# WestlyPark/StyleRenderer

Measured on AMD Instinct MI355X. Metric: generator fwd+bwd images/sec at 256^2, higher is better.
Workload: dtype f32

## Files before the change

### include/stylerenderer_amd.h

```cpp
#ifndef STYLERENDERER_AMD_H_
#define STYLERENDERER_AMD_H_

#include <stddef.h>
#include <stdint.h>

#ifdef __cplusplus
extern "C" {
#endif

typedef void* sr_stream_t;

#define SR_OK 0
#define SR_EINVAL (-1)
#define SR_ERANGE (-2)

const char* sr_error_string(int code);
int sr_abi_version(void);

int sr_fused_bias_act(float* y, const float* x, const float* b, const float* ref, int act, int grad,
                      float alpha, float scale, int64_t size_x, int64_t step_b, int64_t size_b,
                      int use_bias, int use_ref, sr_stream_t stream);

int64_t sr_fused_act_bwd_scratch_floats(int64_t n, int64_t c, int64_t inner);
int sr_fused_act_bwd(float* gx, float* gb, const float* gy, const float* out, float alpha,
// ... 194 lines not shown
                              float eps, sr_stream_t stream);
int sr_rasterize_backward_f64(int64_t b, int64_t n, int64_t h, int64_t w, int repeat_v,
                              int perspective, const double* v, const int64_t* index,
                              double* dcoeff, double eps, sr_stream_t stream);

int64_t sr_rasterize_grad_scratch_bytes(int64_t b, int64_t nf, int64_t tex_c, int is_double);
int sr_rasterize_grad_f32(int64_t b, int64_t nv, int64_t nf, int64_t h, int64_t w, int repeat_f,
                          int perspective, const float* v, const float* tex, int64_t tex_c,
                          const int64_t* tri, const int32_t* win, const int32_t* big, const float* grad_out,
                          const int32_t* adj_off, const int32_t* adj, int64_t adj_off_bstride,
                          int64_t adj_bstride, const int32_t* adj_slot, float* grad_v, float* grad_tex, float eps,
                          void* work, sr_stream_t stream);
int sr_rasterize_grad_f64(int64_t b, int64_t nv, int64_t nf, int64_t h, int64_t w, int repeat_f,
                          int perspective, const double* v, const double* tex, int64_t tex_c,
                          const int64_t* tri, const int32_t* win, const int32_t* big, const double* grad_out,
                          const int32_t* adj_off, const int32_t* adj, int64_t adj_off_bstride,
                          int64_t adj_bstride, const int32_t* adj_slot, double* grad_v, double* grad_tex, double eps,
                          void* work, sr_stream_t stream);

int sr_rasterize_forward_cpu_f32(int64_t b, int64_t nv, int64_t nf, int64_t h, int64_t w, int repeat_v,
                                 int repeat_f, int perspective, const float* v, const int64_t* tri,
                                 int64_t* index, float* coeff, float* zbuf, float eps);
int sr_rasterize_forward_cpu_f64(int64_t b, int64_t nv, int64_t nf, int64_t h, int64_t w, int repeat_v,
                                 int repeat_f, int perspective, const double* v, const int64_t* tri,
                                 int64_t* index, double* coeff, double* zbuf, double eps);
int sr_rasterize_backward_cpu_f32(int64_t b, int64_t n, int64_t h, int64_t w, int perspective,
                                  const float* v, const int64_t* index, float* dcoeff, float eps);
int sr_rasterize_backward_cpu_f64(int64_t b, int64_t n, int64_t h, int64_t w, int perspective,
                                  const double* v, const int64_t* index, double* dcoeff, double eps);

int64_t sr_conv2d_scratch_floats(int64_t B, int64_t C, int64_t N, int64_t IH, int64_t IW, int64_t OH,
                                 int64_t OW, int ksize, int stride, int pad, int transposed);
int sr_conv2d_mfma(float* out, const float* in, const float* wt, const float* iscale,
                   const float* oscale, const float* obias, int64_t B, int64_t C, int64_t N,
                   int64_t wt_ld, int64_t IH, int64_t IW, int64_t OH, int64_t OW, int ksize, int stride,
                   int pad, int transposed, float* scratch, sr_stream_t stream);
int sr_conv2d_nba(float* out, const float* in, const float* wt, const float* iscale, const float* oscale,
                  const float* noise, const float* noise_w, const float* abias, float alpha, float gain, int64_t B,
                  int64_t C, int64_t N, int64_t wt_ld, int64_t H, int64_t W, int64_t noise_bstride, float* scratch,
                  sr_stream_t stream);

#define SR_CONV_U_READY 1
int sr_conv2d_uses_winograd(int64_t B, int64_t C, int64_t N, int64_t IH, int64_t IW, const float* in, const float* out);
#define SR_CONV_PATH_INVALID (-1)
#define SR_CONV_PATH_DIRECT 0
#define SR_CONV_PATH_WINO 1
#define SR_CONV_PATH_S2_BF16 2
#define SR_CONV_PATH_S2_WINO 3
#define SR_CONV_PATH_GEMM1X1 4
#define SR_CONV_PATH_CONVT_TAPS 5
#define SR_CONV_PATH_CONVT_BF16 6
#define SR_CONV_PATH_CONVT_FUSED_KS 7
#define SR_CONV_PATH_CONVT_FUSED 8
#define SR_CONV_PATH_STRIPS 0x100
int sr_conv2d_path(int64_t B, int64_t C, int64_t N, int64_t IH, int64_t IW, int64_t OH, int64_t OW, int ksize, int stride,
                   int pad, int transposed, const float* in, const float* out, const float* wt, int64_t wt_ld,
                   int have_scratch);
int64_t sr_conv2d_path_floats(int64_t B, int64_t C, int64_t N, int64_t IH, int64_t IW, int64_t OH, int64_t OW, int ksize,
                              int stride, int pad, int transposed, const float* in, const float* out, const float* wt,
                              int64_t wt_ld, int have_scratch);

int sr_conv2d_generic(float* y, const float* x, const float* w, const float* bias, int64_t B, int64_t C, int64_t N,
                      int64_t IH, int64_t IW, int64_t OH, int64_t OW, int kh, int kw, int sy, int sx, int py, int px,
                      sr_stream_t stream);
int sr_conv2d_generic_dgrad(float* dx, const float* g, const float* w, int64_t B, int64_t C, int64_t N, int64_t IH,
                            int64_t IW, int64_t OH, int64_t OW, int kh, int kw, int sy, int sx, int py, int px,
                            sr_stream_t stream);
int sr_conv2d_generic_wgrad(float* dw, const float* x, const float* g, int64_t B, int64_t C, int64_t N, int64_t IH,
                            int64_t IW, int64_t OH, int64_t OW, int kh, int kw, int sy, int sx, int py, int px,
                            sr_stream_t stream);
int sr_conv2d_mfma_ex(float* out, const float* in, const float* wt, const float* iscale,
                      const float* oscale, const float* obias, int64_t B, int64_t C, int64_t N,
                      int64_t wt_ld, int64_t IH, int64_t IW, int64_t OH, int64_t OW, int ksize,
                      int stride, int pad, int transposed, int flags, float* scratch, sr_stream_t stream);
int sr_conv1x1_add_supported(int64_t B, int64_t C, int64_t N, int64_t wt_ld, int64_t P, const float* in, const float* wt,
                             const float* out, const float* addend);
int sr_conv1x1_add(float* out, const float* in, const float* wt, const float* oscale, const float* addend, int64_t B,
                   int64_t C, int64_t N, int64_t wt_ld, int64_t P, sr_stream_t stream);
int sr_conv2d_nba_ex(float* out, const float* in, const float* wt, const float* iscale, const float* oscale,
                     const float* noise, const float* noise_w, const float* abias, float alpha, float gain,
                     int64_t B, int64_t C, int64_t N, int64_t wt_ld, int64_t H, int64_t W, int64_t noise_bstride,
                     int flags, float* scratch, sr_stream_t stream);

int64_t sr_conv2d_wgrad_scratch_floats(int64_t B, int64_t C, int64_t N, int64_t IH, int64_t IW,
                                       int64_t OH, int64_t OW, int ksize, int stride, int pad,
                                       int transposed);
int sr_conv2d_wgrad_mfma(float* dwt, const float* x, const float* gy, const float* xscale,
                         const float* gscale, int64_t B, int64_t C, int64_t N, int64_t IH,
                         int64_t IW, int64_t OH, int64_t OW, int ksize, int stride, int pad,
                         int transposed, float* scratch, sr_stream_t stream);
#define SR_WGRAD_PATH_INVALID (-1)
#define SR_WGRAD_PATH_DIRECT 0
#define SR_WGRAD_PATH_SMALL3 1
#define SR_WGRAD_PATH_WINO 2
#define SR_WGRAD_PATH_BF16_1X1 3
#define SR_WGRAD_PATH_BF16_S2 4
#define SR_WGRAD_PATH_S2_DMA 5
#define SR_WGRAD_PATH_S2_WINO 6
int sr_conv2d_wgrad_path(int64_t B, int64_t C, int64_t N, int64_t IH, int64_t IW, int64_t OH, int64_t OW, int ksize,
                         int stride, int pad, int transposed, const float* x, const float* gy);
int64_t sr_conv2d_wgrad_path_floats(int64_t B, int64_t C, int64_t N, int64_t IH, int64_t IW, int64_t OH, int64_t OW,
                                    int ksize, int stride, int pad, int transposed, const float* x, const float* gy);

int sr_signal_bump(uint32_t* counter, sr_stream_t stream);
int sr_signal_set(uint32_t* word, const uint32_t* epoch, sr_stream_t stream);
int sr_signal_wait(const uint32_t* counter, uint32_t at_least, sr_stream_t stream);
// ... 113 lines not shown
```

### stylerenderer_amd/_lib.py

```python
import ctypes
import os

_HERE = os.path.dirname(os.path.abspath(__file__))
LIB_PATH = os.environ.get("STYLERENDERER_AMD_LIB") or os.path.join(_HERE, "libstylerenderer_hip.so")

_i = ctypes.c_int
_l = ctypes.c_int64
_f = ctypes.c_float
_d = ctypes.c_double
_p = ctypes.c_void_p

SIGNATURES = {
    "sr_error_string": (ctypes.c_char_p, [_i]),
    "sr_abi_version": (_i, []),
    "sr_fused_bias_act": (_i, [_p, _p, _p, _p, _i, _i, _f, _f, _l, _l, _l, _i, _i, _p]),
    "sr_fused_act_bwd_scratch_floats": (_l, [_l, _l, _l]),
    "sr_fused_act_bwd": (_i, [_p, _p, _p, _p, _f, _f, _l, _l, _l, _p, _p]),
    "sr_noise_bias_act": (_i, [_p] * 6 + [_f, _f] + [_l] * 4 + [_p]),
    "sr_noise_bias_act_bwd_scratch_floats": (_l, [_l, _l, _l]),
    "sr_noise_bias_act_bwd": (_i, [_p] * 6 + [_f, _f] + [_l] * 4 + [_p, _p]),
    "sr_noise_bias_act_bwd_dot_scratch_floats": (_l, [_l, _l, _l]),
    "sr_noise_bias_act_bwd_dot": (_i, [_p] * 9 + [_f, _f] + [_l] * 4 + [_p, _p]),
    "sr_conv2d_nba": (_i, [_p] * 8 + [_f, _f] + [_l] * 7 + [_p, _p]),
    "sr_conv2d_nba_ex": (_i, [_p] * 8 + [_f, _f] + [_l] * 7 + [_i, _p, _p]),
# ... 89 lines not shown
    "sr_conv2d_mfma_ex": (_i, [_p] * 6 + [_l] * 8 + [_i] * 5 + [_p, _p]),
    "sr_conv1x1_add_supported": (_i, [_l] * 5 + [_p] * 4),
    "sr_conv1x1_add": (_i, [_p] * 5 + [_l] * 5 + [_p]),
    "sr_rasterize_grad_f64": (_i, [_l] * 5 + [_i] * 2 + [_p, _p, _l] + [_p] * 6 + [_l, _l, _p, _p, _p, _d, _p, _p]),
    "sr_pose_fwd": (_i, [_p, _p, _p, _p]),
    "sr_pose_bwd": (_i, [_p, _p, _p, _p, _p]),
    "sr_pose_batch_fwd": (_i, [_p, _p, _p, _l, _p]),
    "sr_affine3_fwd": (_i, [_p, _p, _p, _p, _l, _l, _l, _p]),
    "sr_affine3_bwd": (_i, [_p, _p, _p, _p, _l, _l, _l, _p]),
    "sr_morph_fwd": (_i, [_p] * 9 + [_f, _l, _l, _l, _p]),
    "sr_vertex_normals_bwd_f32": (_i, [_p] * 11 + [_l, _l, _l, _f, _p]),
    "sr_morph_gcoeff_scratch_floats": (_l, [_l, _l, _l]),
    "sr_morph_gcoeff": (_i, [_p] * 6 + [_f, _p, _l, _l, _l, _p]),
    "sr_morph_pose_bwd": (_i, [_p] * 5 + [_l, _p]),
    "sr_skin_joints_fwd": (_i, [_p] * 11 + [_f] + [_l] * 4 + [_p]),
    "sr_skin_fwd": (_i, [_p] * 7 + [_l] * 4 + [_p]),
    "sr_skin_bwd_scratch_floats": (_l, [_l, _l, _l]),
    "sr_skin_bwd": (_i, [_p] * 7 + [_l] * 3 + [_p]),
    "sr_skin_joints_bwd": (_i, [_p] * 11 + [_f, _p] + [_l] * 5 + [_p]),
    "sr_blend_z_floats": (_l, [_l, _l, _l]),
    "sr_blend_head": (_i, [_p] * 6 + [_f] + [_l] * 3 + [_p]),
    "sr_blend_fwd": (_i, [_p] * 8 + [_l] * 4 + [_p]),
    "sr_blend_gz": (_i, [_p] * 3 + [_l] * 4 + [_p]),
    "sr_blend_tail": (_i, [_p] * 5 + [_f, _p] + [_l] * 3 + [_p]),
    "sr_resample_u8_scratch_bytes": (_l, [_l] * 6 + [ctypes.POINTER(ctypes.c_int32)] + [_l] * 4),
    "sr_resample_u8": (_i, [_p, _p] + [_l] * 6 + [_p, _p, ctypes.POINTER(ctypes.c_int32), _l] * 2 + [_l] * 4
                       + [_i, _i, _p, _p]),
    "sr_warp_affine_u8": (_i, [_p, _p, _p] + [_l] * 7 + [_i, _i, _i, _p]),
    "sr_landmark_loss_fwd": (_i, [_p] * 8 + [_l] * 5 + [_f, _f, _p]),
    "sr_landmark_loss_bwd": (_i, [_p, _p, _p, _l, _p, _p, _p] + [_l] * 5 + [_i, _p]),
    "sr_landmark_dyn_fwd": (_i, [_p] * 15 + [_l] * 6 + [_i, _f, _f, _l, _l, _f, _f, _p]),
    "sr_landmark_dyn_bwd": (_i, [_p, _p, _p, _l] + [_p] * 7 + [_l] * 6 + [_i, _p]),
    "sr_region_fill": (_i, [_p, _p, _p] + [_l] * 6 + [_p]),
    "sr_region_grow": (_i, [_p, _p, _l, _l, _l, _i, _p]),
    "sr_region_blend_fwd": (_i, [_p] * 6 + [_l] * 4 + [_f] + [_l] * 4 + [_p]),
    "sr_region_blend_bwd": (_i, [_p] * 3 + [_l] * 4 + [_p]),
    "sr_texture_bake": (_i, [_p] * 9 + [_l] * 10 + [_f, _f, _f, _p]),
    "sr_texture_pad": (_i, [_p] * 4 + [_l] * 4 + [_p]),
    "sr_texture_merge": (_i, [_p] * 5 + [_l] * 4 + [_i, _p]),
    "sr_share_rows": (_i, [_p] + [_l] * 3 + [_p]),
    "sr_camera_fwd": (_i, [_p] * 5 + [_l, _l, _p]),
    "sr_camera_bwd": (_i, [_p] * 6 + [_l, _l, _p]),
    "sr_signal_bump": (_i, [_p, _p]),
    "sr_signal_wait": (_i, [_p, ctypes.c_uint32, _p]),
    "sr_signal_set": (_i, [_p, _p, _p]),
    "sr_signal_set_host": (_i, [_p, _p, _p]),
    "sr_signal_wait_timeout": (_i, [_p, ctypes.c_uint32, ctypes.c_uint64, _p, _i, _p]),
    "sr_signal_wait_poison": (_i, [_p, ctypes.c_uint32, ctypes.c_uint64, _p, _i, _p, _p]),
    "sr_graph_replace_memset_nodes": (_i, [_p, ctypes.POINTER(_i)]),
    "sr_graph_node_count": (_i, [_p, ctypes.POINTER(_i), ctypes.POINTER(_i)]),
}

(CONV_PATH_DIRECT, CONV_PATH_WINO, CONV_PATH_S2_BF16, CONV_PATH_S2_WINO, CONV_PATH_GEMM1X1, CONV_PATH_CONVT_TAPS,
 CONV_PATH_CONVT_BF16, CONV_PATH_CONVT_FUSED_KS, CONV_PATH_CONVT_FUSED) = range(9)
CONV_PATH_STRIPS = 0x100
(WGRAD_PATH_DIRECT, WGRAD_PATH_SMALL3, WGRAD_PATH_WINO, WGRAD_PATH_BF16_1X1, WGRAD_PATH_BF16_S2,
 WGRAD_PATH_S2_DMA, WGRAD_PATH_S2_WINO) = range(7)

_lib = None


class NativeLibraryError(RuntimeError):
    pass


def lib():
    global _lib
    if _lib is not None:
        return _lib
    if not os.path.isfile(LIB_PATH):
        raise NativeLibraryError(
            "stylerenderer_amd: %s not found. Build it with `python -c 'import __graft_entry__ as g; "
            "g.build()'` (hipcc --offload-arch=gfx950). There is no CPU/PyTorch fallback for device "
            "tensors." % LIB_PATH)
    try:
        handle = ctypes.CDLL(LIB_PATH)
    except OSError as e:
        raise NativeLibraryError("stylerenderer_amd: cannot load %s: %s" % (LIB_PATH, e))
    for name, (res, args) in SIGNATURES.items():
        try:
            fn = getattr(handle, name)
        except AttributeError:
            raise NativeLibraryError("stylerenderer_amd: %s does not export %s" % (LIB_PATH, name))
        fn.restype = res
        fn.argtypes = args
    _lib = handle
    return _lib


def check(rc, what=""):
    if rc != 0:
        msg = lib().sr_error_string(rc)
        raise RuntimeError("%s failed: %s (code %d)" % (what or "stylerenderer_amd call",
                                                        msg.decode() if msg else "?", rc))


def ptr(t):
    if t is None or t.numel() == 0:
        return None
    return t.data_ptr()


def current_stream(device=None):
    import torch

    return torch.cuda.current_stream(device).cuda_stream
```

### stylerenderer_amd/build.py

```python
import os
import subprocess
import sys

HERE = os.path.dirname(os.path.abspath(__file__))
CSRC = os.path.join(HERE, "csrc")
LIB = os.path.join(HERE, "libstylerenderer_hip.so")
OBJ = os.path.join(HERE, "csrc", "_obj")

ARCH = "gfx950"
COMMON = ["--offload-arch=" + ARCH, "-O3", "-std=c++17", "-fPIC", "-Wno-unused-result",
          "-fhip-fp32-correctly-rounded-divide-sqrt"]
EXACT = ["-ffp-contract=off"]
NOSLP = ["-fno-slp-vectorize"]

SOURCES = [
    ("capi.hip", EXACT),
    ("fused_bias_act.hip", EXACT),
    ("upfirdn2d.hip", EXACT + NOSLP),
    ("rasterize.hip", EXACT),
    ("fused_elem.hip", EXACT),
    ("weight_prep.hip", EXACT),
    ("style_linear.hip", EXACT),
    ("bank_mm.hip", EXACT),
    ("mesh.hip", EXACT),
    ("landmark.hip", EXACT),
    ("region.hip", EXACT),
    ("texture.hip", EXACT),
    ("share.hip", EXACT),
    ("camera.hip", EXACT),
    ("morph.hip", []),
    ("skin.hip", []),
    ("blend.hip", []),
    ("lpips.hip", EXACT),
    ("ppl.hip", EXACT),
    ("augment.hip", EXACT),
    ("resample.hip", EXACT),
    ("warp.hip", EXACT),
    ("conv_mfma.hip", []),
    ("conv_wino.hip", []),
    ("conv_wgrad_wino.hip", []),
    ("conv_wgrad_mfma.hip", []),
    ("conv_wgrad_bf16x3.hip", []),
    ("conv_wgrad_s2_wino.hip", []),
    ("conv_s2_bf16x3.hip", []),
    ("conv_s2_wino.hip", []),
    ("conv_generic.hip", []),
    ("conv1x1_gemm.hip", []),
    ("inception.hip", []),
]


def _hipcc():
    for c in (os.environ.get("HIPCC"), "/opt/rocm/bin/hipcc", "hipcc"):
        if c and (os.path.isabs(c) and os.path.exists(c) or not os.path.isabs(c)):
            return c
    return "hipcc"


def _deps(src):
    deps = [src, os.path.join(CSRC, "common.h"),
            os.path.join(HERE, "..", "include", "stylerenderer_amd.h"), os.path.abspath(__file__)]
    deps += [os.path.join(CSRC, f) for f in os.listdir(CSRC) if f.endswith(".h")]
    return max(os.path.getmtime(d) for d in deps if os.path.exists(d))


def build_library(force=False, verbose=False):
    os.makedirs(OBJ, exist_ok=True)
    hipcc = _hipcc()
    objs, rebuilt = [], False
    procs = []
    for name, extra in SOURCES:
        src = os.path.join(CSRC, name)
        obj = os.path.join(OBJ, name.replace(".hip", ".o"))
        objs.append(obj)
        if force or not os.path.exists(obj) or os.path.getmtime(obj) < _deps(src):
            cmd = [hipcc] + COMMON + extra + ["-c", src, "-o", obj]
            if verbose:
                print(" ".join(cmd))
            procs.append((name, subprocess.Popen(cmd, stdout=subprocess.PIPE, stderr=subprocess.STDOUT)))
            rebuilt = True
    for name, p in procs:
        out, _ = p.communicate()
        if p.returncode != 0:
            sys.stderr.write(out.decode(errors="replace"))
            raise RuntimeError("hipcc failed on %s" % name)
        if verbose and out:
            sys.stdout.write(out.decode(errors="replace"))
    if rebuilt or not os.path.exists(LIB):
        cmd = [hipcc, "--offload-arch=" + ARCH, "-shared", "-fPIC", "-o", LIB] + objs
        if verbose:
            print(" ".join(cmd))
        subprocess.check_call(cmd)
    return LIB


if __name__ == "__main__":
    print(build_library(force="-f" in sys.argv, verbose=True))
```

### stylerenderer_amd/csrc/conv_mfma.hip

```cpp
#include "common.h"
#include "conv1x1_gemm.h"
#include "conv_s2_bf16x3.h"
#include "conv_s2_wino.h"
#include "conv_wgrad_bf16x3.h"
#include "conv_wino.h"

#include <algorithm>
#include <cstdlib>

namespace {

typedef float f32x16 __attribute__((ext_vector_type(16)));
typedef const void __attribute__((address_space(1)))* gptr_t;
typedef void __attribute__((address_space(3)))* lptr_t;

constexpr int BN = 128;
constexpr int BM = 128;

__device__ __attribute__((aligned(16))) const float g_zero_line[4] = {0.f, 0.f, 0.f, 0.f};
__device__ __attribute__((aligned(16))) const float g_ones_line[4] = {1.f, 1.f, 1.f, 1.f};

struct ConvParams {
    const float* in;
    const float* wt;
    const float* iscale;
    const float* oscale;
    const float* obias;
    float* out;
    int B, C, N, ldw;
    int IH, IW;
    int GH, GW;
    int gy_base, gx_base;
    int OH, OW;
    int osy, osx, ooy, oox;
    int dy0, dx0;
    int wmap[9];
    int tiles_x, tiles_y, tiles_b, tiles_n;
    float* partial;
    int64_t partial_floats;
    int ks, c_per_slice;
    int tap_first, tap_step, tap_count;
};

template <int IS, int TY, int TX, int PW, int PH, int PB, bool V4, bool TAP9 = false>
struct Geo {
    static constexpr bool ROT = V4 && IS == 2;
    static constexpr int NT = TY * TX;
    static constexpr int KC = NT >= 9 ? 4 : (NT >= 4 ? 8 : 16);
    static constexpr int EH = (PH - 1) * IS + TY;
    static constexpr int EW = (PW - 1) * IS + TX;
    static constexpr int LEAD = (V4 && !ROT) ? (TAP9 ? 4 : (TX > 1 ? 3 : 0)) : 0;
    static constexpr int EWP = ROT ? (EW + 3 + 3) / 4 * 4
                                   : (V4 ? (LEAD + EW + 3) / 4 * 4 : EW + ((EW % 2 == 0) ? 1 : 0));
    static constexpr int PLANE = PB * EH * EWP;
    static constexpr int W_FLOATS = NT * KC * BN;
    static constexpr int W_INSTR = W_FLOATS / 256;
    static constexpr int IMG_INSTR = V4 ? (KC * PLANE + 255) / 256 : 0;
    static constexpr int ST_INSTR = V4 ? (KC * PB + 63) / 64 : 0;
// ... 813 lines not shown
    if (ext_w <= 0 || ext_h <= 0) return SR_OK;
    choose_split(ext_h, ext_w, p.B, p.N, p.C, p.ks, p.c_per_slice);
    if (!p.partial || (int64_t)p.ks * p.B * p.N * ext_h * ext_w > p.partial_floats) {
        p.ks = 1;
        p.c_per_slice = (p.C + 15) / 16 * 16;
    }
    patch_shape(ext_w, pw, ph, pb);
    p.tiles_x = (ext_w + pw - 1) / pw;
    p.tiles_y = (ext_h + ph - 1) / ph;
    p.tiles_b = (p.B + pb - 1) / pb;
    p.tiles_n = (p.N + BN - 1) / BN;
    const int64_t blocks = (int64_t)p.tiles_x * p.tiles_y * p.tiles_b * p.tiles_n * p.ks;
    if (blocks <= 0) return SR_OK;
    if (blocks > 0x7FFFFFFFLL) return SR_ERANGE;
    const dim3 grid((unsigned)blocks);
    const bool v4 = IS == 1 && pb == 1 && p.IW % 4 == 0 && sr_aligned16(p.in) &&
                    p.gx_base % 4 == 0 && p.dx0 == (TX > 1 ? -1 : 0);
    const bool rot = IS == 2 && pb == 1 && (p.IW & 3) == 1 && ((p.IH * p.IW) & 3) == 1 && p.C % 4 == 0 &&
                     sr_aligned16(p.in) && p.dx0 >= 0 && p.dy0 >= 0 && p.gx_base == 0 &&
                     p.gy_base == 0 && (p.GW - 1) * 2 + p.dx0 + TX <= p.IW && (p.GH - 1) * 2 + p.dy0 + TY <= p.IH &&
                     ext_w % pw == 0 && ext_h % ph == 0 && !sr_env_off("SR_CONV_ROT");
    int rc;
    if (IS == 1 && v4) {
        if (pw == 32) rc = launch_one<1, TY, TX, 32, 4, 1, true>(p, grid, st);
        else rc = launch_one<1, TY, TX, 16, 8, 1, true>(p, grid, st);
    } else if (IS == 2 && rot && TY == 3 && TX == 3) {
        if (pw == 32) rc = launch_one<2, 3, 3, 32, 4, 1, true>(p, grid, st);
        else rc = launch_one<2, 3, 3, 16, 8, 1, true>(p, grid, st);
    } else if (pw == 32) rc = launch_one<IS, TY, TX, 32, 4, 1, false>(p, grid, st);
    else if (pw == 16) rc = launch_one<IS, TY, TX, 16, 8, 1, false>(p, grid, st);
    else if (pw == 8) rc = launch_one<IS, TY, TX, 8, 8, 2, false>(p, grid, st);
    else rc = launch_one<IS, TY, TX, 4, 4, 8, false>(p, grid, st);
    if (rc != SR_OK || p.ks <= 1) return rc;
    const int64_t total = (int64_t)p.B * p.N * ext_h * ext_w;
    hipLaunchKernelGGL(k_conv_reduce, dim3(sr_stream_grid(total, 256)), dim3(256), 0, st, p, ext_h, ext_w);
    return sr_launch_status();
}


int64_t direct_floats(const ConvCall& c) {
    int ks, per;
    int64_t need = 0;
    auto consider = [&](int64_t gh, int64_t gw) {
        if (gh <= 0 || gw <= 0) return;
        choose_split((int)gh, (int)gw, (int)c.B, (int)c.N, (int)c.C, ks, per);
        if (ks > 1) need = std::max(need, ks * c.B * c.N * gh * gw);
    };
    if (!c.transposed) consider(c.OH, c.OW);
    else consider(c.IH + 1, c.IW + 1), consider(c.IH, c.IW), consider(1, c.IW + 1), consider(c.IH, 1);
    return need;
}

bool convt_interior(int path) {
    return path == SR_CONV_PATH_CONVT_BF16 || path == SR_CONV_PATH_CONVT_FUSED_KS || path == SR_CONV_PATH_CONVT_FUSED;
}

struct ConvPlan {
    int path = SR_CONV_PATH_DIRECT;
    bool strips = false;
    int ks = 1, c_per_slice = 0;
    bool taps_gemm = false;
    int64_t floats = 0;
    int64_t sized = 0;
    int code() const { return path | (strips ? SR_CONV_PATH_STRIPS : 0); }
};

ConvPlan make_conv_plan(const ConvCall& c, bool have_scratch) {
    ConvPlan plan;
    const int64_t B = c.B, C = c.C, N = c.N, IH = c.IH, IW = c.IW, OH = c.OH, OW = c.OW;
    if (B <= 0 || C <= 0 || N <= 0 || OH <= 0 || OW <= 0) return plan;
    plan.sized = plan.floats = direct_floats(c);
    auto candidate = [&](int path, bool reach, bool take, int64_t floats, int ks = 1) {
        if (!reach) return;
        plan.sized = std::max(plan.sized, floats);
        if (plan.path != SR_CONV_PATH_DIRECT || !take || (floats > 0 && !have_scratch)) return;
        plan.path = path; plan.floats = floats; plan.ks = ks;
    };
    if (!c.transposed && c.is3x3(1, 1)) {
        if (sr_winograd_enabled() && sr_wino_eligible(B, C, N, IH, IW, nullptr, nullptr))
            candidate(SR_CONV_PATH_WINO, true, sr_wino_eligible(B, C, N, IH, IW, c.in, c.out),
                      sr_wino_scratch_floats(C, N) + sr_wino_partial_floats(B, C, N, IH, IW));
    } else if (!c.transposed && c.is3x3(2, 0)) {
        candidate(SR_CONV_PATH_S2_BF16, sr_wgrad_bf16x3_enabled('c') && sr_conv_s2_bf16x3_eligible(B, C, N, IH, IW, OH, OW),
                  true, sr_conv_s2_bf16x3_scratch_floats(C, N));
        const int sw = sr_env_char("SR_CONV_S2_WINO");
        candidate(SR_CONV_PATH_S2_WINO, sr_conv_s2_wino_eligible(B, C, N, IH, IW, OH, OW, nullptr, nullptr),
                  sw != '0' && sr_conv_s2_wino_eligible(B, C, N, IH, IW, OH, OW, c.in, c.out) &&
                      (sw == 'f' || sr_conv_s2_wino_blocks(B, N, OH, OW) >= S2_WINO_MIN_BLOCKS),
                  sr_conv_s2_wino_scratch_floats(C, N));
    } else if (!c.transposed && c.ksize == 1 && c.stride == 1) {
        candidate(SR_CONV_PATH_GEMM1X1, true,
                  c.pad == 0 && sr_conv1x1_gemm_eligible(B, C, N, c.ldw, IH * IW, c.in, c.wt, c.out), 0);
    } else if (c.transposed && c.is3x3(2, 0)) {
        const bool bf = sr_wgrad_bf16x3_enabled('t') && sr_convt_bf16x3_eligible(B, C, N, IH, IW);
        if (convt_taps_wanted(B, C, N, IH, IW)) {
            int ks;
            convt_taps_plan((int)IH, (int)IW, (int)B, (int)N, (int)C, ks, plan.c_per_slice);
            candidate(SR_CONV_PATH_CONVT_TAPS, true, !bf, (int64_t)ks * 9 * B * N * (IH + 1) * (IW + 1), ks);
        }
        candidate(SR_CONV_PATH_CONVT_BF16, bf, true, sr_convt_bf16x3_scratch_floats(C, N));
        const int sw = sr_env_char("SR_CONVT_FUSED");
        const bool fused_ok = sw != '0' && IW >= 16 && convt_fused_eligible(c);
        const int64_t blocks = (IW / TFused::PW) * (IH / TFused::PH) * ((N + BN - 1) / BN) * B;
        const bool pays = blocks >= 192 || C <= 256;
        const int ks = (IW % TFused::PW || IH % TFused::PH || pays) ? 1 : convt_fused_slices(blocks, (int)C);
        candidate(SR_CONV_PATH_CONVT_FUSED_KS, ks > 1, fused_ok && !sr_env_off("SR_CONVT_FUSED_KS"),
                  ks * B * N * (2 * IH + 1) * (2 * IW + 1), ks);
        candidate(SR_CONV_PATH_CONVT_FUSED, true, fused_ok && (pays || sw == '1'), 0);
        const int64_t strip = convt_strip_floats(B, N, IH, IW);
        plan.sized = std::max(plan.sized, strip);
        if (convt_interior(plan.path) && have_scratch && !sr_env_off("SR_CONVT_STRIPS")) {
            plan.strips = true;
            plan.floats = std::max(plan.floats, strip);
        }
    }
    if (plan.path == SR_CONV_PATH_CONVT_TAPS)
        plan.taps_gemm = sr_convt_taps_gemm_eligible(B, C, N, IW, c.ldw, plan.c_per_slice, c.wt);
    return plan;
}

bool conv_call_valid(const ConvCall& c) {
    if (c.B < 0 || c.C <= 0 || c.N <= 0 || c.IH <= 0 || c.IW <= 0 || c.OH <= 0 || c.OW <= 0) return false;
    if (c.transposed) return c.is3x3(2, 0) && c.OH == 2 * c.IH + 1 && c.OW == 2 * c.IW + 1;
    return (c.ksize == 3 || c.ksize == 1) && (c.stride == 1 || c.stride == 2) &&
           c.OH == (c.IH + 2 * c.pad - c.ksize) / c.stride + 1 && c.OW == (c.IW + 2 * c.pad - c.ksize) / c.stride + 1;
}

int launch_convt_phases(ConvParams p, bool interior_done, hipStream_t st) {
    for (int py = 0; py < 2; ++py)
        for (int px = 0; px < 2; ++px) {
            const int TYp = py == 0 ? 2 : 1, TXp = px == 0 ? 2 : 1;
            p.osy = p.osx = 2; p.ooy = py; p.oox = px;
            p.dy0 = -(TYp - 1); p.dx0 = -(TXp - 1);
            for (int ty = 0; ty < TYp; ++ty)
                for (int tx = 0; tx < TXp; ++tx) {
                    const int ky = py + 2 * (TYp - 1 - ty), kx = px + 2 * (TXp - 1 - tx);
                    p.wmap[ty * TXp + tx] = ky * 3 + kx;
                }
            const int gh_full = py == 0 ? p.IH + 1 : p.IH, gw_full = px == 0 ? p.IW + 1 : p.IW;
            int regions[3][4] = {{0, p.IH, 0, p.IW},
                                 {p.IH, gh_full, 0, gw_full},
                                 {0, p.IH, p.IW, gw_full}};
            const bool split_border = p.IW >= 16;
            if (!split_border) {
                regions[0][1] = gh_full;
                regions[0][3] = gw_full;
            }
            const bool fused = split_border && interior_done;
            for (int rg = fused ? 1 : 0; rg < (split_border ? 3 : 1); ++rg) {
                p.gy_base = regions[rg][0]; p.GH = regions[rg][1];
                p.gx_base = regions[rg][2]; p.GW = regions[rg][3];
                if (p.GH <= p.gy_base || p.GW <= p.gx_base) continue;
                int rc;
                if (py == 0 && px == 0) rc = launch_by_patch<1, 2, 2>(p, st);
// ... 25 lines not shown
extern "C" int64_t sr_conv2d_path_floats(int64_t B, int64_t C, int64_t N, int64_t IH, int64_t IW, int64_t OH, int64_t OW,
                                         int ksize, int stride, int pad, int transposed, const float* in, const float* out,
                                         const float* wt, int64_t wt_ld, int have_scratch) {
    const ConvCall c{B, C, N, IH, IW, OH, OW, ksize, stride, pad, transposed, in, out, wt, wt_ld};
    return conv_call_valid(c) ? make_conv_plan(c, have_scratch != 0).floats : -1;
}

extern "C" int sr_conv2d_uses_winograd(int64_t B, int64_t C, int64_t N, int64_t IH, int64_t IW, const float* in,
                                       const float* out) {
    return make_conv_plan(ConvCall{B, C, N, IH, IW, IH, IW, 3, 1, 1, 0, in, out, nullptr, 0}, true).path == SR_CONV_PATH_WINO;
}

extern "C" int sr_conv2d_mfma_ex(float* out, const float* in, const float* wt, const float* iscale,
                              const float* oscale, const float* obias, int64_t B, int64_t C,
                              int64_t N, int64_t wt_ld, int64_t IH, int64_t IW, int64_t OH, int64_t OW,
                              int ksize, int stride, int pad, int transposed, int flags, float* scratch,
                              sr_stream_t stream) {
    const ConvCall c{B, C, N, IH, IW, OH, OW, ksize, stride, pad, transposed, in, out, wt, wt_ld};
    if (B < 0 || C <= 0 || N <= 0 || IH <= 0 || IW <= 0 || OH <= 0 || OW <= 0) return SR_EINVAL;
    if (wt_ld < N || wt_ld % 4 != 0 || !sr_aligned16(wt)) return SR_EINVAL;
    if (B == 0) return SR_OK;
    if (!out || !in || !wt) return SR_EINVAL;
    if (B * C * IH * IW >= (1LL << 31) || B * N * OH * OW >= (1LL << 40) ||
        (int64_t)ksize * ksize * C * wt_ld >= (1LL << 31))
        return SR_ERANGE;
    if (!conv_call_valid(c)) return SR_EINVAL;
    const ConvPlan plan = make_conv_plan(c, scratch != nullptr);
    hipStream_t st = sr_stream(stream);
    ConvParams p;
    p.in = in; p.wt = wt; p.iscale = iscale; p.oscale = oscale; p.obias = obias; p.out = out;
    p.B = (int)B; p.C = (int)C; p.N = (int)N; p.ldw = (int)wt_ld;
    p.IH = (int)IH; p.IW = (int)IW; p.OH = (int)OH; p.OW = (int)OW;
    p.partial = scratch;
    p.partial_floats = scratch ? plan.sized : 0;
    for (int i = 0; i < 9; ++i) p.wmap[i] = 0;
    p.ks = 1; p.c_per_slice = (p.C + 15) / 16 * 16;
    p.tap_first = 0; p.tap_step = 1; p.tap_count = 9;
    int rc = SR_OK;
    switch (plan.path) {
    case SR_CONV_PATH_WINO:
        return sr_wino_conv3x3(out, in, wt, wt_ld, iscale, oscale, obias, B, C, N, IH, IW, scratch, st, nullptr,
                               (flags & SR_CONV_U_READY) != 0);
    case SR_CONV_PATH_S2_BF16:
        return sr_conv_s2_bf16x3_launch(out, in, wt, wt_ld, iscale, oscale, obias, B, C, N, IH, IW, OH, OW, scratch, st);
    case SR_CONV_PATH_S2_WINO:
        return sr_conv_s2_wino_launch(out, in, wt, wt_ld, iscale, oscale, obias, B, C, N, IH, IW, OH, OW, scratch, st);
    case SR_CONV_PATH_GEMM1X1:
        return sr_conv1x1_gemm_launch(out, in, wt, wt_ld, iscale, oscale, obias, B, C, N, IH * IW, st);
    case SR_CONV_PATH_CONVT_TAPS:
        return launch_convt_taps(p, plan.ks, plan.c_per_slice, plan.taps_gemm, st);
    case SR_CONV_PATH_CONVT_BF16:
        rc = sr_convt_bf16x3_launch(out, in, wt, wt_ld, iscale, oscale, obias, B, C, N, IH, IW, scratch, st);
        break;
    case SR_CONV_PATH_CONVT_FUSED_KS:
    case SR_CONV_PATH_CONVT_FUSED:
        for (int i = 0; i < 9; ++i) p.wmap[i] = i;
        rc = launch_convt_fused(p, plan.ks, st);
        break;
    default:
        if (transposed) break;
        p.GH = p.OH; p.GW = p.OW;
        p.gy_base = p.gx_base = 0;
        p.osy = p.osx = 1; p.ooy = p.oox = 0;
        p.dy0 = p.dx0 = -pad;
        for (int i = 0; i < ksize * ksize; ++i) p.wmap[i] = i;
        if (ksize == 3) return stride == 1 ? launch_by_patch<1, 3, 3>(p, st) : launch_by_patch<2, 3, 3>(p, st);
        return stride == 1 ? launch_by_patch<1, 1, 1>(p, st) : launch_by_patch<2, 1, 1>(p, st);
    }
    if (rc != SR_OK) return rc;
    if (plan.strips) return launch_convt_strips(p, st);
    return launch_convt_phases(p, convt_interior(plan.path), st);
}

extern "C" int sr_conv2d_mfma(float* out, const float* in, const float* wt, const float* iscale,
                              const float* oscale, const float* obias, int64_t B, int64_t C,
                              int64_t N, int64_t wt_ld, int64_t IH, int64_t IW, int64_t OH, int64_t OW,
                              int ksize, int stride, int pad, int transposed, float* scratch,
                              sr_stream_t stream) {
    return sr_conv2d_mfma_ex(out, in, wt, iscale, oscale, obias, B, C, N, wt_ld, IH, IW, OH, OW, ksize, stride, pad,
                             transposed, 0, scratch, stream);
}

extern "C" int sr_conv2d_nba_ex(float* out, const float* in, const float* wt, const float* iscale, const float* oscale,
                                const float* noise, const float* noise_w, const float* abias, float alpha, float gain,
                                int64_t B, int64_t C, int64_t N, int64_t wt_ld, int64_t H, int64_t W,
                                int64_t noise_bstride, int flags, float* scratch, sr_stream_t stream) {
    if (B < 0 || C <= 0 || N <= 0 || H <= 0 || W <= 0) return SR_EINVAL;
    if (wt_ld < N || wt_ld % 4 != 0 || !sr_aligned16(wt)) return SR_EINVAL;
    if (B == 0) return SR_OK;
    if (!out || !in || !wt || !scratch || (noise && !noise_w)) return SR_EINVAL;
    if (!sr_conv2d_uses_winograd(B, C, N, H, W, in, out)) return SR_EINVAL;
    const WinoNba nba{noise, noise_w, abias, noise_bstride, alpha, gain};
    return sr_wino_conv3x3(out, in, wt, wt_ld, iscale, oscale, nullptr, B, C, N, H, W, scratch, sr_stream(stream), &nba,
                           (flags & SR_CONV_U_READY) != 0);
}

extern "C" int sr_conv2d_nba(float* out, const float* in, const float* wt, const float* iscale, const float* oscale,
                             const float* noise, const float* noise_w, const float* abias, float alpha, float gain,
                             int64_t B, int64_t C, int64_t N, int64_t wt_ld, int64_t H, int64_t W,
                             int64_t noise_bstride, float* scratch, sr_stream_t stream) {
    return sr_conv2d_nba_ex(out, in, wt, iscale, oscale, noise, noise_w, abias, alpha, gain, B, C, N, wt_ld, H, W,
                            noise_bstride, 0, scratch, stream);
}
```

Measured before the change: 583.1.

## Add Winograd-style MFMA kernel for stride-2 transposed 3x3 convolutions

Introduces a new transposed-conv path that splits the stride-2 3x3 transposed convolution into even/odd output-row parity halves and applies a 1D Winograd-like transform along x (and across rows for even parity), reducing the multiplies fed to f32 MFMA. Inputs and weights are streamed into LDS via buffer_load_lds with double buffering, and epilogue scaling and bias are fused into the store. The planner selects it for large problems (above a FLOP threshold) when eligible, taking priority over the fused and taps paths. Risks include numerical differences from the transform and extra LDS pressure limiting occupancy.

```diff
diff --git a/include/stylerenderer_amd.h b/include/stylerenderer_amd.h
--- a/include/stylerenderer_amd.h
+++ b/include/stylerenderer_amd.h
@@ -270,6 +270,7 @@
 #define SR_CONV_PATH_CONVT_BF16 6
 #define SR_CONV_PATH_CONVT_FUSED_KS 7
 #define SR_CONV_PATH_CONVT_FUSED 8
+#define SR_CONV_PATH_CONVT_WINO 9
 #define SR_CONV_PATH_STRIPS 0x100
 int sr_conv2d_path(int64_t B, int64_t C, int64_t N, int64_t IH, int64_t IW, int64_t OH, int64_t OW, int ksize, int stride,
                    int pad, int transposed, const float* in, const float* out, const float* wt, int64_t wt_ld,
diff --git a/stylerenderer_amd/_lib.py b/stylerenderer_amd/_lib.py
--- a/stylerenderer_amd/_lib.py
+++ b/stylerenderer_amd/_lib.py
@@ -165,7 +165,7 @@
 }
 
 (CONV_PATH_DIRECT, CONV_PATH_WINO, CONV_PATH_S2_BF16, CONV_PATH_S2_WINO, CONV_PATH_GEMM1X1, CONV_PATH_CONVT_TAPS,
- CONV_PATH_CONVT_BF16, CONV_PATH_CONVT_FUSED_KS, CONV_PATH_CONVT_FUSED) = range(9)
+ CONV_PATH_CONVT_BF16, CONV_PATH_CONVT_FUSED_KS, CONV_PATH_CONVT_FUSED, CONV_PATH_CONVT_WINO) = range(10)
 CONV_PATH_STRIPS = 0x100
 (WGRAD_PATH_DIRECT, WGRAD_PATH_SMALL3, WGRAD_PATH_WINO, WGRAD_PATH_BF16_1X1, WGRAD_PATH_BF16_S2,
  WGRAD_PATH_S2_DMA, WGRAD_PATH_S2_WINO) = range(7)
diff --git a/stylerenderer_amd/build.py b/stylerenderer_amd/build.py
--- a/stylerenderer_amd/build.py
+++ b/stylerenderer_amd/build.py
@@ -44,6 +44,7 @@
     ("conv_wgrad_s2_wino.hip", []),
     ("conv_s2_bf16x3.hip", []),
     ("conv_s2_wino.hip", []),
+    ("convt_wino.hip", []),
     ("conv_generic.hip", []),
     ("conv1x1_gemm.hip", []),
     ("inception.hip", []),
diff --git a/stylerenderer_amd/csrc/conv_mfma.hip b/stylerenderer_amd/csrc/conv_mfma.hip
--- a/stylerenderer_amd/csrc/conv_mfma.hip
+++ b/stylerenderer_amd/csrc/conv_mfma.hip
@@ -4,6 +4,7 @@
 #include "conv_s2_wino.h"
 #include "conv_wgrad_bf16x3.h"
 #include "conv_wino.h"
+#include "convt_wino.h"
 
 #include <algorithm>
 #include <cstdlib>
@@ -923,8 +924,12 @@
 }
 
 bool convt_interior(int path) {
-    return path == SR_CONV_PATH_CONVT_BF16 || path == SR_CONV_PATH_CONVT_FUSED_KS || path == SR_CONV_PATH_CONVT_FUSED;
-}
+    return path == SR_CONV_PATH_CONVT_BF16 || path == SR_CONV_PATH_CONVT_WINO || path == SR_CONV_PATH_CONVT_FUSED_KS ||
+           path == SR_CONV_PATH_CONVT_FUSED;
+}
+
+constexpr double CONVT_WINO_MIN_FLOPS = 4.0e10;
+static_assert(CONVT_WINO_MIN_FLOPS > 18.0 * 8 * 512 * 512 * 32 * 32, "the t3s2 row of tests/conv_plan_cases.py stays on k_convt_fused");
 
 struct ConvPlan {
     int path = SR_CONV_PATH_DIRECT;
@@ -964,13 +969,18 @@
                   c.pad == 0 && sr_conv1x1_gemm_eligible(B, C, N, c.ldw, IH * IW, c.in, c.wt, c.out), 0);
     } else if (c.transposed && c.is3x3(2, 0)) {
         const bool bf = sr_wgrad_bf16x3_enabled('t') && sr_convt_bf16x3_eligible(B, C, N, IH, IW);
+        const int sw = sr_env_char("SR_CONVT_FUSED"), wsw = sr_env_char("SR_CONVT_WINO");
+        const bool wino_ok = sw != '0' && wsw != '0' && sr_convt_wino_eligible(B, C, N, IH, IW, c.ldw, c.in);
+        const bool wino_forced = wino_ok && wsw == 'f' && !bf;
         if (convt_taps_wanted(B, C, N, IH, IW)) {
             int ks;
             convt_taps_plan((int)IH, (int)IW, (int)B, (int)N, (int)C, ks, plan.c_per_slice);
-            candidate(SR_CONV_PATH_CONVT_TAPS, true, !bf, (int64_t)ks * 9 * B * N * (IH + 1) * (IW + 1), ks);
+            candidate(SR_CONV_PATH_CONVT_TAPS, true, !bf && !wino_forced, (int64_t)ks * 9 * B * N * (IH + 1) * (IW + 1), ks);
         }
         candidate(SR_CONV_PATH_CONVT_BF16, bf, true, sr_convt_bf16x3_scratch_floats(C, N));
-        const int sw = sr_env_char("SR_CONVT_FUSED");
+        candidate(SR_CONV_PATH_CONVT_WINO, sr_convt_wino_eligible(B, C, N, IH, IW, c.ldw, nullptr),
+                  wino_ok && (wsw == 'f' || 18.0 * (double)B * (double)C * (double)N * (double)IH * (double)IW >=
+                                                CONVT_WINO_MIN_FLOPS), 0);
         const bool fused_ok = sw != '0' && IW >= 16 && convt_fused_eligible(c);
         const int64_t blocks = (IW / TFused::PW) * (IH / TFused::PH) * ((N + BN - 1) / BN) * B;
         const bool pays = blocks >= 192 || C <= 256;
@@ -1102,6 +1112,9 @@
     case SR_CONV_PATH_CONVT_BF16:
         rc = sr_convt_bf16x3_launch(out, in, wt, wt_ld, iscale, oscale, obias, B, C, N, IH, IW, scratch, st);
         break;
+    case SR_CONV_PATH_CONVT_WINO:
+        rc = sr_convt_wino_launch(out, in, wt, wt_ld, iscale, oscale, obias, B, C, N, IH, IW, st);
+        break;
     case SR_CONV_PATH_CONVT_FUSED_KS:
     case SR_CONV_PATH_CONVT_FUSED:
         for (int i = 0; i < 9; ++i) p.wmap[i] = i;
diff --git a/stylerenderer_amd/csrc/convt_wino.h b/stylerenderer_amd/csrc/convt_wino.h
--- /dev/null
+++ b/stylerenderer_amd/csrc/convt_wino.h
@@ -0,0 +1,8 @@
+#pragma once
+#include <hip/hip_runtime.h>
+#include <stdint.h>
+
+bool sr_convt_wino_eligible(int64_t B, int64_t C, int64_t N, int64_t IH, int64_t IW, int64_t ldw, const void* in);
+int sr_convt_wino_launch(float* out, const float* in, const float* wt, int64_t ldw, const float* iscale,
+                         const float* oscale, const float* obias, int64_t B, int64_t C, int64_t N, int64_t IH,
+                         int64_t IW, hipStream_t st);
diff --git a/stylerenderer_amd/csrc/convt_wino.hip b/stylerenderer_amd/csrc/convt_wino.hip
--- /dev/null
+++ b/stylerenderer_amd/csrc/convt_wino.hip
@@ -0,0 +1,287 @@
+#include "common.h"
+#include "convt_wino.h"
+
+namespace {
+
+typedef float f32x16 __attribute__((ext_vector_type(16)));
+typedef void __attribute__((address_space(3)))* lptr_t;
+
+constexpr int KC = 8;
+constexpr int NB = 64;
+constexpr int PW = 32, PH = 8;
+constexpr int LEAD = 3;
+constexpr int EWP = LEAD + 1 + PW;
+constexpr int EH = PH + 1;
+constexpr int PLANE = EH * EWP;
+constexpr int I_INSTR = (KC * PLANE / 4 + 63) / 64;
+constexpr int I_FLOATS = I_INSTR * 256;
+constexpr int I_PER_WAVE = (I_INSTR + 3) / 4;
+constexpr int BUF = I_FLOATS + 9 * KC * NB;
+constexpr int PAD = 2 * BUF;
+constexpr int STY = PAD + 4 * 256;
+static_assert(PLANE % 4 == 0 && EWP % 4 == 0, "16-byte DMA pieces must not straddle a row");
+
+struct ConvtWinoParams {
+    const float* in;
+    const float* wt;
+    const float* iscale;
+    const float* oscale;
+    const float* obias;
+    float* out;
+    int B, C, N, ldw, IH, IW, OH, OW;
+    int tiles_x, tiles_y, tiles_n;
+    int half_blocks;
+};
+
+template <int PAR>
+__device__ __forceinline__ void convt_wino_body(const ConvtWinoParams& p, float* smem, int bid) {
+#if __HIP_DEVICE_COMPILE__
+    constexpr int NR = PAR ? 2 : 3;
+    constexpr int NWR = PAR ? 1 : 3;
+    constexpr int NTAP = PAR ? 3 : 9, TAP0 = PAR ? 3 : 0;
+    constexpr int NM = NR * 5;
+    constexpr int W_INSTR = NTAP * KC * NB / 256;
+    constexpr int W_PER_WAVE = (W_INSTR + 3) / 4;
+    constexpr int N_DMA = I_PER_WAVE + W_PER_WAVE;
+    static_assert(N_DMA > 4 && N_DMA <= 8, "DMA slots: four behind the barrier, the rest in the first k-step");
+    float* const sty = smem + STY;
+
+    {
+        const int nwg = p.half_blocks;
+        const int q = nwg / SR_NUM_XCD, r = nwg % SR_NUM_XCD, xcd = bid % SR_NUM_XCD;
+        bid = (xcd < r ? xcd * (q + 1) : r * (q + 1) + (xcd - r) * q) + bid / SR_NUM_XCD;
+    }
+    const int n_t = bid % p.tiles_n;
+    bid /= p.tiles_n;
+    const int tx_i = bid % p.tiles_x;
+    bid /= p.tiles_x;
+    const int ty_i = bid % p.tiles_y;
+    const int b = bid / p.tiles_y;
+    const int n0 = n_t * NB, j0 = ty_i * PH, i0 = tx_i * PW;
+
+    const int tid = threadIdx.x, lane = tid & 63;
+    const int wave = __builtin_amdgcn_readfirstlane(tid >> 6);
+    const int half = lane >> 5, l31 = lane & 31;
+    const int wn = wave & 1, wt = wave >> 1;
+    const int ty_l = wt * 2 + (l31 >> 4), tx_l = l31 & 15;
+
+    constexpr int OOB = 0x7FFFFFF0;
+    int i_off[I_PER_WAVE], w_off[W_PER_WAVE];
+#pragma unroll
+    for (int i = 0; i < I_PER_WAVE; ++i) {
+        const int j = wave + 4 * i;
+        const int f = (j * 64 + lane) * 4;
+        int off = OOB;
+        if (j < I_INSTR && f < KC * PLANE) {
+            const int c = f / PLANE, q = f % PLANE;
+            const int r = q / EWP, cola = q % EWP;
+            const int gy = j0 - 1 + r, gx = i0 - 4 + cola;
+            if (gy >= 0 && gy < p.IH && gx >= 0 && gx + 3 < p.IW) off = ((c * p.IH + gy) * p.IW + gx) * 4;
+        }
+        i_off[i] = off;
+    }
+#pragma unroll
+    for (int i = 0; i < W_PER_WAVE; ++i) {
+        const int j = wave + 4 * i;
+        const int row = 4 * j + (lane >> 4);
+        const int t = TAP0 + row / KC, c = row % KC;
+        w_off[i] = j < W_INSTR ? ((t * p.C + c) * p.ldw + n0 + (lane & 15) * 4) * 4 : OOB;
+    }
+    const int plane_in = p.IH * p.IW;
+    const __amdgpu_buffer_rsrc_t r_w = uniform_rsrc(p.wt, 9 * p.C * p.ldw * 4);
+    const __amdgpu_buffer_rsrc_t r_in = uniform_rsrc(p.in + (int64_t)b * p.C * plane_in, p.C * plane_in * 4);
+    const int nchunks = p.C / KC;
+
+    auto dma1 = [&](int k, int i) {
+        const int kc = min(k, nchunks - 1), c0 = kc * KC;
+        float* dst = smem + (k & 1) * BUF;
+        if (i < I_PER_WAVE) {
+            const int j = wave + 4 * i;
+            __builtin_amdgcn_raw_ptr_buffer_load_lds(r_in, (lptr_t)(j < I_INSTR ? dst + j * 256 : smem + PAD + wave * 256),
+                                                     16, i_off[i], c0 * plane_in * 4, 0, 0);
+        } else {
+            const int ii = i - I_PER_WAVE, j = wave + 4 * ii;
+            __builtin_amdgcn_raw_ptr_buffer_load_lds(
+                r_w, (lptr_t)(j < W_INSTR ? dst + I_FLOATS + j * 256 : smem + PAD + wave * 256), 16, w_off[ii],
+                c0 * p.ldw * 4, 0, 0);
+        }
+    };
+
+    f32x16 acc[NR][5];
+#pragma unroll
+    for (int i = 0; i < NR; ++i)
+#pragma unroll
+        for (int j = 0; j < 5; ++j)
+#pragma unroll
+            for (int r = 0; r < 16; ++r) acc[i][j][r] = 0.0f;
+
+    const int x_off = half * PLANE + (2 * ty_l + (PAR ? 1 : 0)) * EWP + LEAD + 2 * tx_l;
+    const int a_off = I_FLOATS + half * NB + wn * 32 + l31;
+
+#pragma unroll
+    for (int i = 0; i < N_DMA; ++i) dma1(0, i);
+#pragma unroll
+    for (int i = 0; i < 4; ++i) dma1(1, i);
+    for (int c = tid; c < p.C; c += 256) sty[c] = p.iscale ? p.iscale[(int64_t)b * p.C + c] : 1.0f;
+    __builtin_amdgcn_s_waitcnt(0x0F70);
+    __syncthreads();
+
+    float RX[NR][3], RA[NWR][3], T0[NR];
+    float X[2][NR][4], A[2][NWR][4];
+    float sc_next;
+    auto load_raw = [&](const float* sb, int c0, int cp) {
+#pragma unroll
+        for (int r = 0; r < NR; ++r)
+#pragma unroll
+            for (int cx = 0; cx < 3; ++cx) RX[r][cx] = sb[(2 * cp) * PLANE + x_off + r * EWP + cx];
+#pragma unroll
+        for (int r = 0; r < NWR; ++r)
+#pragma unroll
+            for (int kx = 0; kx < 3; ++kx) RA[r][kx] = sb[((r * 3 + kx) * KC + 2 * cp) * NB + a_off];
+        sc_next = sty[c0 + 2 * cp + half];
+    };
+    auto xform = [&](int m, int s) {
+        if (m >= 1 && m <= 3) {
+            const int cx = m - 1;
+            float v[NR];
+            if constexpr (PAR == 0) {
+                v[1] = RX[1][cx] * sc_next;
+                v[0] = __builtin_fmaf(RX[0][cx], sc_next, -v[1]);
+                v[2] = __builtin_fmaf(RX[2][cx], sc_next, -v[1]);
+            } else {
+                v[0] = RX[0][cx] * sc_next;
+                v[1] = RX[1][cx] * sc_next;
+            }
+#pragma unroll
+            for (int r = 0; r < NR; ++r) {
+                if (cx == 0) T0[r] = v[r];
+                else if (cx == 1) X[s][r][1] = v[r];
+                else X[s][r][3] = v[r];
+            }
+        } else if (m >= 4 && m < 4 + NR) {
+            const int r = m - 4;
+            X[s][r][0] = T0[r] - X[s][r][1];
+            X[s][r][2] = X[s][r][3] - X[s][r][1];
+        } else if constexpr (PAR == 0) {
+            if (m == 7) {
+#pragma unroll
+                for (int kx = 0; kx < 3; ++kx) {
+                    const float lo = RA[0][kx], hi = RA[2][kx];
+                    const int q = kx == 0 ? 2 : (kx == 1 ? 3 : 0);
+                    A[s][0][q] = hi;
+                    A[s][2][q] = lo;
+                    A[s][1][q] = lo + hi;
+                }
+            } else if (m == 8) {
+#pragma unroll
+                for (int r = 0; r < 3; ++r) A[s][r][1] = A[s][r][0] + A[s][r][2];
+            }
+        } else if (m == 6) {
+            A[s][0][0] = RA[0][2];
+            A[s][0][2] = RA[0][0];
+            A[s][0][3] = RA[0][1];
+            A[s][0][1] = RA[0][0] + RA[0][2];
+        }
+    };
+    load_raw(smem, 0, 0);
+#pragma unroll
+    for (int m = 0; m < NM; ++m) xform(m, 0);
+
+    for (int k = 0; k < nchunks; ++k) {
+        const float* sb = smem + (k & 1) * BUF;
+        const float* sbn = smem + ((k + 1) & 1) * BUF;
+        const int c0 = k * KC, c0n = min(k + 1, nchunks - 1) * KC;
+#pragma unroll
+        for (int cp = 0; cp < KC / 2; ++cp) {
+            const int cur = cp & 1, nxt = cur ^ 1;
+            if (cp == KC / 2 - 1) {
+                __builtin_amdgcn_s_waitcnt(0x0F70);
+                __syncthreads();
+                load_raw(sbn, c0n, 0);
+            } else {
+                load_raw(sb, c0, cp + 1);
+            }
+            __builtin_amdgcn_sched_barrier(0);
+#pragma unroll
+            for (int m = 0; m < NM; ++m) {
+                constexpr int CV[5] = {0, 1, 2, 1, 3}, CW[5] = {0, 1, 2, 3, 3};
+                const int rp = m / 5, q = m % 5;
+                acc[rp][q] = __builtin_amdgcn_mfma_f32_32x32x2f32(A[cur][PAR ? 0 : rp][CW[q]], X[cur][rp][CV[q]], acc[rp][q],
+                                                                  0, 0, 0);
+                xform(m, nxt);
+                if (m >= NM - 5 && m < NM - 1) {
+                    const int u = m - (NM - 5);
+                    if (cp == 0 && 4 + u < N_DMA) dma1(k + 1, 4 + u);
+                    else if (cp == KC / 2 - 1) dma1(k + 2, u);
+                }
+                __builtin_amdgcn_sched_barrier(0);
+            }
+        }
+    }
+    __builtin_amdgcn_s_waitcnt(0x0F70);
+
+    const int64_t plane_out = (int64_t)p.OH * p.OW;
+    const int Y0 = 2 * j0 + 4 * ty_l, X0 = 2 * i0 + 4 * tx_l;
+#pragma unroll
+    for (int r = 0; r < 16; ++r) {
+        const int n = n0 + wn * 32 + (r & 3) + 8 * (r >> 2) + 4 * half;
+        const float os = p.oscale ? p.oscale[(int64_t)b * p.N + n] : 1.0f;
+        const float ob = p.obias ? p.obias[n] : 0.0f;
+        float* o = p.out + ((int64_t)b * p.N + n) * plane_out + (int64_t)Y0 * p.OW + X0;
+#pragma unroll
+        for (int yr = 0; yr < 2; ++yr) {
+            float v[5];
+#pragma unroll
+            for (int q = 0; q < 5; ++q) {
+                if constexpr (PAR == 0) v[q] = acc[yr ? 2 : 0][q][r] + acc[1][q][r];
+                else v[q] = acc[yr][q][r];
+            }
+            float* orow = o + (int64_t)(2 * yr + PAR) * p.OW;
+            orow[0] = (v[0] + v[1]) * os + ob;
+            orow[1] = v[3] * os + ob;
+            orow[2] = (v[2] + v[1]) * os + ob;
+            orow[3] = v[4] * os + ob;
+        }
+    }
+#endif
+}
+
+__global__ __launch_bounds__(256) void k_convt_wino(const ConvtWinoParams p) {
+    extern __shared__ __attribute__((aligned(16))) float smem[];
+    const int bid = blockIdx.x;
+    if (bid < p.half_blocks) convt_wino_body<0>(p, smem, bid);
+    else convt_wino_body<1>(p, smem, bid - p.half_blocks);
+}
+
+}
+
+bool sr_convt_wino_eligible(int64_t B, int64_t C, int64_t N, int64_t IH, int64_t IW, int64_t ldw, const void* in) {
+    if (B <= 0 || C <= 0 || N <= 0 || IH <= 0 || IW <= 0) return false;
+    if (IW % PW != 0 || IH % PH != 0 || C % KC != 0 || C > 2048 || N % NB != 0) return false;
+    if (C * IH * IW >= (1LL << 29) - 4 || 9 * C * ldw >= (1LL << 29) - 4) return false;
+    if (2 * B * (IW / PW) * (IH / PH) * (N / NB) > 0x7FFFFFFFLL) return false;
+    return sr_aligned16(in);
+}
+
+int sr_convt_wino_launch(float* out, const float* in, const float* wt, int64_t ldw, const float* iscale,
+                         const float* oscale, const float* obias, int64_t B, int64_t C, int64_t N, int64_t IH,
+                         int64_t IW, hipStream_t st) {
+    ConvtWinoParams p;
+    p.in = in; p.wt = wt; p.iscale = iscale; p.oscale = oscale; p.obias = obias; p.out = out;
+    p.B = (int)B; p.C = (int)C; p.N = (int)N; p.ldw = (int)ldw;
+    p.IH = (int)IH; p.IW = (int)IW; p.OH = 2 * (int)IH + 1; p.OW = 2 * (int)IW + 1;
+    p.tiles_x = (int)(IW / PW); p.tiles_y = (int)(IH / PH); p.tiles_n = (int)(N / NB);
+    p.half_blocks = p.tiles_x * p.tiles_y * p.tiles_n * p.B;
+    const int lds = (STY + (int)C) * 4;
+    static bool configured = false;
+    if (!configured) {
+        if (hipFuncSetAttribute(reinterpret_cast<const void*>(k_convt_wino), hipFuncAttributeMaxDynamicSharedMemorySize,
+                                160 * 1024) != hipSuccess) {
+            (void)hipGetLastError();
+            return SR_EINVAL;
+        }
+        configured = true;
+    }
+    hipLaunchKernelGGL(k_convt_wino, dim3(2u * (unsigned)p.half_blocks), dim3(256), lds, st, p);
+    return sr_launch_status();
+}
```

Measured after the change: 597.5 (median of 6 runs). 1.02x the previous value.
